# kelaendi/mused

Hardware: AMD Instinct MI355X
Metric: stream rows/sec, d=1024 l=128 window=10k synthetic (SWFD + kNN similarity + eigenstep + labels) (higher is better)
Workload: dtype f64; 1 GPU; synthetic d=1024 l=128 window=10000 k=50 (BASELINE config 2); stream=blob, W=10000, d=1024, l=128, k=50, modalities=1, swfd_levels=14, rccl_ranks=1, lanes_per_gpu=20, padded_window_slots=2

## Files before the change

mused_amd/csrc/swfd.hip:

```cpp
#include <vector>

#include "internal.h"

namespace mused {

struct Swfd {
  int N, d, ell, L, S, cap, n2, n4, n3;
  int lanes;
  double R;
  long i;
  int pend;
  long restart_mark;
  int skip_dead;
  bool twin;
  int sweeps;
  double* buf;
  double* queue;
  long long* qt;
  int* meta;
  int* rep;
  int* list;
  int* offs;
  int oround;
  int* kact;
  long long* ostat;
  long long* dropped;
  double* theta;
  double *T, *Wc;
  int gram_split;
  double* gpart;
  int* plan;
  int* keep_src;
  long long* now_dev;
  int* status;
  int* status_host;
  EigPlan* eig;
  double *stack, *Wq, *Bout, *sig_out, *qinfo;
  int* qsel;
  EigPlan* eigq;
  EigPlan* eigq3;
  int pre_chunk;
  double *pre_in, *pre_out, *pre_gram;
  EigPlan* eigp;
};

static inline int sk_index(const Swfd* h, int lane, int level, int kind) { return lane * 2 * h->L + kind * h->L + level; }

struct BitWord { unsigned long long w; };
template <typename T>
__device__ __forceinline__ double row_elem(const T* row, int c) { return (double)row[c]; }
template <>
__device__ __forceinline__ double row_elem<BitWord>(const BitWord* row, int c) {
  return (double)((row[c >> 6].w >> (c & 63)) & 1ull);
}

template <typename T>
__global__ void swfd_append_kernel(const T* __restrict__ X, long ldx, long lane_stride, int per_lane, int m, int d,
                                   int n2, int pend, const int* __restrict__ meta, double* __restrict__ buf) {
  const int r = blockIdx.x, s = blockIdx.y;
  X += (long)(s / per_lane) * lane_stride;
  const int row = meta[s * 4 + 0] + pend + r;
  if (row >= n2) return;
  double* dst = buf + ((long)s * n2 + row) * d;
  const T* src = X + (long)r * ldx;
  for (int c = threadIdx.x; c < d; c += blockDim.x) dst[c] = row_elem<T>(src, c);
}

__global__ void swfd_restart_kernel(double* __restrict__ buf, double* __restrict__ queue, long long* __restrict__ qt,
                                    int* __restrict__ meta, long long* __restrict__ dropped, int L, long buf_elems,
                                    long queue_elems, int cap) {
  const int lane = blockIdx.y / L, j = blockIdx.y - lane * L;
  const int sm = lane * 2 * L + j, sa = sm + L;
  const long gid = (long)blockIdx.x * blockDim.x + threadIdx.x;
  if (gid < buf_elems) {
    buf[sm * buf_elems + gid] = buf[sa * buf_elems + gid];
    buf[sa * buf_elems + gid] = 0.0;
  }
  if (gid < queue_elems) queue[sm * queue_elems + gid] = queue[sa * queue_elems + gid];
  if (gid < cap) qt[sm * cap + gid] = qt[sa * cap + gid];
  if (gid == 0) {
    for (int k = 0; k < 4; ++k) {
      meta[sm * 4 + k] = meta[sa * 4 + k];
      meta[sa * 4 + k] = 0;
    }
    dropped[sm] = dropped[sa];
    dropped[sa] = 0;
  }
}

__global__ void swfd_set_now_kernel(long long* now, long long v) { *now = v; }

constexpr int SWFD_OFFS_ROUND = 16;
__global__ __launch_bounds__(1024) void swfd_rep_kernel(const int* __restrict__ meta, int L, int nchains, int* __restrict__ rep,
                                                        int twin, const long long* __restrict__ dropped, long long epoch_start,
                                                        int skip_dead, long long* __restrict__ now_dev, long long now, int pend,
                                                        int ell, int n2, int* __restrict__ list, int* __restrict__ offs,
                                                        int* __restrict__ kact, long long* __restrict__ ostat, int oround) {
  extern __shared__ int s_key[];
  __shared__ int s_hist[17];
  const int t = threadIdx.x, S = nchains * L;
  if (t == 0) *now_dev = now;
  if (t < 17) s_hist[t] = 0;
  auto put = [&](int s, int r) {
    rep[s] = r;
    const int na = meta[s * 4 + 0] + pend;
    s_key[s] = (r == s) ? (na < n2 ? na : n2) : -1;
  };
  for (int c = t; c < nchains; c += 1024) {
    const int base = ((twin && (c & 1)) ? c - 1 : c) * L;
    if (twin && (c & 1)) {
      int r = base + L - 1;
      put(c * L + L - 1, r);
      for (int j = L - 2; j >= 0; --j) {
        if (meta[(base + j) * 4 + 3] != 0) r = base + j;
        put(c * L + j, r);
      }
      continue;
    }
    const bool dead_ok = skip_dead && !twin && (c & 1) == 0;
    int r = base + L - 1;
    put(r, r);
    for (int j = L - 2; j >= 0; --j) {
      if (meta[(base + j) * 4 + 3] != 0) r = base + j;
      put(base + j, (dead_ok && dropped[base + j] > epoch_start) ? -1 : r);
    }
  }
  __syncthreads();
  if (!list) return;
  for (int s = t; s < S; s += 1024) {
    const int key = s_key[s];
    if (key < 0) continue;
    int rank = 0;
    for (int j = 0; j < S; ++j) {
      const int kj = s_key[j];
      rank += (kj > key) || (kj == key && j < s);
    }
    list[1 + rank] = s;
    const int n = offs ? n2 - ((n2 - (key > ell ? key : ell)) & ~(oround - 1)) : n2;
    if (offs) offs[s] = n2 - n;
    if (kact) kact[s] = min(n2, (key + 15) & ~15);
    atomicAdd(&s_hist[16], 1);
    atomicAdd(&s_hist[(n - 1) >> 4 < 16 ? (n - 1) >> 4 : 15], 1);
  }
  __syncthreads();
  if (t == 0) list[0] = s_hist[16];
  if (t == 0) ostat[0] += 1;
  if (t == 1) ostat[1] += s_hist[16];
  if (t < 16) ostat[2 + t] += s_hist[t];
}

__global__ __launch_bounds__(1024) void swfd_decide_kernel(const double* __restrict__ evals,
                                                          const double* __restrict__ U, int ldu, int n2,
                                                          int ell, int cap,
                                                          int N, const long long* __restrict__ now_p,
                                                          const double* __restrict__ theta, int* __restrict__ meta,
                                                          long long* __restrict__ qt, long long* __restrict__ dropped,
                                                          int* __restrict__ plan, int* __restrict__ keep_src,
                                                          double* __restrict__ Wc, const int* __restrict__ rep) {
  __shared__ double lam[1024];
  __shared__ int order[1024];
  __shared__ double scale[512];
  const int s = blockIdx.x, t = threadIdx.x;
  const long long now = *now_p;
  const int sr = rep ? rep[s] : s;
  if (sr < 0) return;
  const double* ev = evals + (long)sr * ldu;
  const double* Us = U + (long)sr * ldu * ldu;
  if (t < n2) lam[t] = ev[t];
  __syncthreads();
  if (t < n2) {
    const double mine = lam[t];
    int rank = 0;
    for (int j = 0; j < n2; ++j) {
      const double o = lam[j];
      rank += (o > mine) || (o == mine && j < t);
    }
    order[rank] = t;
  }
  __syncthreads();
  __shared__ int s_part[16];
  __shared__ int s_wcnt[3][4];
  const int head0 = meta[s * 4 + 1], cnt0 = meta[s * 4 + 2];
  long long* q = qt + (long)s * cap;
  const int wv = t >> 6, ln = t & 63;
  int expired = 0;
  for (int k = t; k < cnt0; k += 1024) expired += (q[(head0 + k) % cap] + N <= now) ? 1 : 0;
#pragma unroll
  for (int o = 32; o > 0; o >>= 1) expired += __shfl_xor(expired, o);
  if (ln == 0) s_part[wv] = expired;
  __syncthreads();
  int nexp = 0;
#pragma unroll
  for (int ww = 0; ww < 16; ++ww) nexp += s_part[ww];
  const int head1 = (head0 + nexp) % cap, cnt1 = cnt0 - nexp;
  const double l0 = lam[order[0]];
  const double delta = lam[order[ell - 1]] > 0.0 ? lam[order[ell - 1]] : 0.0;
  const double tol = 1e-10 * (l0 > 0.0 ? l0 : 0.0);
  const double th = theta[s];
  int kind = 0, near = 0;
  double sc = 0.0;
  if (t < ell) {
    const double l = lam[order[t]];
    double s2 = l - delta;
    s2 = s2 > 0.0 ? s2 : 0.0;
    if (s2 > tol) {
      sc = sqrt(s2 / l) / l;
      kind = (s2 >= th) ? 2 : 1;
      near = (kind == 2 && s2 < 2.0 * th) ? 1 : 0;
    }
    scale[t] = sc;
  }
  const unsigned long long mk = __ballot(kind == 1), md = __ballot(kind == 2), mn = __ballot(near != 0);
  const unsigned long long below = (ln == 0) ? 0ull : (~0ull >> (64 - ln));
  if (ln == 0 && wv < 4) {
    s_wcnt[0][wv] = __popcll(mk);
    s_wcnt[1][wv] = __popcll(md);
    s_wcnt[2][wv] = __popcll(mn);
  }
  __syncthreads();
  int kpos = __popcll(mk & below), dpos = __popcll(md & below);
  int nk = 0, nd = 0, nnear = 0;
#pragma unroll
  for (int ww = 0; ww < 4; ++ww) {
    if (ww < wv) {
      kpos += s_wcnt[0][ww];
      dpos += s_wcnt[1][ww];
    }
    nk += s_wcnt[0][ww];
    nd += s_wcnt[1][ww];
    nnear += s_wcnt[2][ww];
  }
  const int nevict = (cnt1 + nd > cap) ? (cnt1 + nd - cap) : 0;
  if (t == 0) {
    long long drop = dropped[s];
    if (nevict > 0) {
      const long long ts = q[(head1 + nevict - 1) % cap];
      drop = ts > drop ? ts : drop;
    }
    dropped[s] = drop;
  }
  __syncthreads();
  if (t < ell) {
    int pos = 0;
    if (kind == 1) {
      pos = kpos;
      keep_src[s * ell + kpos] = t;
    } else if (kind == 2) {
      pos = (head1 + cnt1 + dpos) % cap;
      q[pos] = now;
    }
    plan[(s * ell + t) * 2 + 0] = kind;
    plan[(s * ell + t) * 2 + 1] = pos;
  }
  if (t == 0) {
    meta[s * 4 + 0] = nk;
    meta[s * 4 + 1] = (head1 + nevict) % cap;
    meta[s * 4 + 2] = cnt1 + nd - nevict;
    meta[s * 4 + 3] += nnear;
  }
  __syncthreads();
  if (sr != s) return;
  double* W = Wc + (long)s * ell * n2;
  for (int e = t; e < ell * n2; e += 1024) {
    const int i = e / n2, a = e - i * n2;
    const double sc = scale[i];
    W[e] = (sc != 0.0) ? sc * Us[(long)order[i] * ldu + a] : 0.0;
  }
}

__global__ void swfd_scatter_kernel(const double* __restrict__ T, const int* __restrict__ plan,
                                    const int* __restrict__ keep_src, const int* __restrict__ meta,
                                    double* __restrict__ buf, double* __restrict__ queue, int n2, int ell, int cap,
                                    int d, const int* __restrict__ rep) {
  const int rho = blockIdx.x, s = blockIdx.y;
  if (rep && rep[s] < 0) return;
  const double* Ts = T + (long)(rep ? rep[s] : s) * ell * d;
  if (rho < ell && plan[(s * ell + rho) * 2] == 2) {
    const int slot = plan[(s * ell + rho) * 2 + 1];
    double* dst = queue + ((long)s * cap + slot) * d;
    const double* src = Ts + (long)rho * d;
    for (int c = threadIdx.x; c < d; c += blockDim.x) dst[c] = src[c];
  }
  const int nk = meta[s * 4 + 0];
  double* dst = buf + ((long)s * n2 + rho) * d;
  if (rho < nk) {
    const double* src = Ts + (long)keep_src[s * ell + rho] * d;
    for (int c = threadIdx.x; c < d; c += blockDim.x) dst[c] = src[c];
  } else {
    for (int c = threadIdx.x; c < d; c += blockDim.x) dst[c] = 0.0;
  }
}

static int swfd_rotate_all(Swfd* h, hipStream_t st) {
  const int S = h->S, n2 = h->n2, d = h->d, ell = h->ell;
  int rc;
  if (h->rep)
    hipLaunchKernelGGL(swfd_rep_kernel, dim3(1), dim3(1024), sizeof(int) * (size_t)S, st, h->meta, h->L, 2 * h->lanes, h->rep,
                       h->twin ? 1 : 0, h->dropped, (long long)(((h->i - 1) / h->N) * h->N), h->skip_dead, h->now_dev,
                       (long long)h->i, h->pend, ell, n2, h->list, h->offs, h->kact, h->ostat, h->oround);
  else
    hipLaunchKernelGGL(swfd_set_now_kernel, dim3(1), dim3(1), 0, st, h->now_dev, (long long)h->i);
  if (h->gram_split > 1) {
    const int kchunk = ((d + h->gram_split - 1) / h->gram_split + 15) / 16 * 16;
    if ((rc = gemm_f64_batched_splitk(true, true, h->buf, d, (long)n2 * d, h->buf, d, (long)n2 * d, h->gpart, n2, n2, d, S, kchunk,
                                      h->gram_split, st, h->rep, h->list)))
      return rc;
    if ((rc = gemm_batched_splitk_reduce(h->gpart, h->gram_split, (long)n2 * n2, eig_plan_input(h->eig), S, h->rep, st, h->list)))
      return rc;
  } else if ((rc = gemm_f64(true, true, h->buf, d, (long)n2 * d, h->buf, d, (long)n2 * d, eig_plan_input(h->eig), n2,
                            (long)n2 * n2, n2, n2, d, S, 1.0, st, h->rep, h->list)))
    return rc;
  if ((rc = eig_plan_run_inplace(h->eig, nullptr, nullptr, st, true))) return rc;
  const EigColumns e = eig_plan_columns(h->eig);
  hipLaunchKernelGGL(swfd_decide_kernel, dim3(S), dim3(1024), 0, st, e.lam, e.cols, e.ld, n2, ell, h->cap, h->N, h->now_dev,
                     h->theta, h->meta, h->qt, h->dropped, h->plan, h->keep_src, h->Wc, h->rep);
  if ((rc = gemm_f64(true, false, h->Wc, n2, (long)ell * n2, h->buf, d, (long)n2 * d, h->T, d, (long)ell * d, ell, d,
                     n2, S, 1.0, st, h->rep, h->list, h->kact)))
    return rc;
  hipLaunchKernelGGL(swfd_scatter_kernel, dim3(n2, S), dim3(256), 0, st, h->T, h->plan, h->keep_src, h->meta, h->buf,
                     h->queue, n2, ell, h->cap, d, h->rep);
  MUSED_LAUNCH_CHECK();
  h->pend = 0;
  return MUSED_OK;
}

static int swfd_restart(Swfd* h, hipStream_t st) {
  const long be = (long)h->n2 * h->d, qe = (long)h->cap * h->d;
  const long m = be > qe ? be : qe;
  hipLaunchKernelGGL(swfd_restart_kernel, dim3(cdiv(m, 256), h->L * h->lanes), dim3(256), 0, st, h->buf, h->queue, h->qt,
                     h->meta, h->dropped, h->L, be, qe, h->cap);
  MUSED_LAUNCH_CHECK();
  return MUSED_OK;
}

constexpr int SWFD_PRE_MAX = 96;
struct PreBlocks {
  int row0[SWFD_PRE_MAX];
  int rows[SWFD_PRE_MAX];
};

template <typename T>
__global__ void swfd_pre_load_kernel(const T* __restrict__ X, long ldx, long lane_stride, int lanes, int ell, int d,
                                     PreBlocks pb, double* __restrict__ out) {
  const int row = blockIdx.x, z = blockIdx.y;
  const int blk = z / lanes, lane = z - blk * lanes;
  double* dst = out + ((long)z * ell + row) * d;
  if (row < pb.rows[blk]) {
    const T* src = X + (long)lane * lane_stride + (long)(pb.row0[blk] + row) * ldx;
    for (int c = threadIdx.x; c < d; c += blockDim.x) dst[c] = row_elem<T>(src, c);
  } else {
    for (int c = threadIdx.x; c < d; c += blockDim.x) dst[c] = 0.0;
  }
}

__global__ void swfd_pre_pack_kernel(const double* __restrict__ gram, int ell, double* __restrict__ Gc) {
  const int n2 = 2 * ell;
  const long z = blockIdx.y;
  const long e = (long)blockIdx.x * blockDim.x + threadIdx.x;
  if (e >= (long)n2 * n2) return;
  const int col = (int)(e / n2), row = (int)(e - (long)col * n2);
  double v = 0.0;
  if (col < ell) v = (row < ell) ? gram[z * ell * ell + (long)col * ell + row] : ((row - ell == col) ? 1.0 : 0.0);
  Gc[z * n2 * n2 + e] = v;
}

template <typename T>
static int swfd_prerotate(Swfd* h, const T* X, long ldx, long lane_stride, const PreBlocks& pb, int nblk, hipStream_t st) {
  const int ell = h->ell, d = h->d, B = h->lanes, n2 = h->n2;
  int rc;
  const int Z = nblk * B;
  hipLaunchKernelGGL(swfd_pre_load_kernel<T>, dim3(ell, Z), dim3(256), 0, st, X, ldx, lane_stride, B, ell, d, pb,
                     h->pre_in);
  if ((rc = gemm_f64(true, true, h->pre_in, d, (long)ell * d, h->pre_in, d, (long)ell * d, h->pre_gram, ell,
                     (long)ell * ell, ell, ell, d, Z, 1.0, st)))
    return rc;
  hipLaunchKernelGGL(swfd_pre_pack_kernel, dim3(cdiv((long)n2 * n2, 256), Z), dim3(256), 0, st, h->pre_gram, ell,
                     eig_plan_input(h->eigp));
  if ((rc = eig_plan_run_inplace(h->eigp, nullptr, nullptr, st, true))) return rc;
  const double* cols = eig_plan_columns(h->eigp).cols;
  const int ld = eig_plan_columns(h->eigp).ld;
  if ((rc = gemm_f64(true, false, cols + ell, ld, (long)ld * ld, h->pre_in, d, (long)ell * d, h->pre_out, d, (long)ell * d,
                     ell, d, ell, Z, 1.0, st)))
    return rc;
  MUSED_LAUNCH_CHECK();
  return MUSED_OK;
}

template <typename T>
static int swfd_append_t(Swfd* h, const T* X, long ldx, long lane_stride, long m, hipStream_t st) {
  long r = 0;
  int rc;
  PreBlocks pb;
  int pre_n = 0, pre_next = 0;
  while (r < m) {
    if (h->i > 0 && h->i % h->N == 0 && h->restart_mark != h->i) {
      if ((rc = swfd_restart(h, st))) return rc;
      h->restart_mark = h->i;
      h->twin = false;
    }
    const long in_epoch = h->i % h->N;
    long until = h->ell - (in_epoch % h->ell);
    if (h->N - in_epoch < until) until = h->N - in_epoch;
    const long take = (m - r) < until ? (m - r) : until;
    bool from_pre = false;
    if (h->pre_chunk > 0 && h->pend == 0 && take == until) {
      if (pre_next >= pre_n) {
        pre_n = pre_next = 0;
        long rr = r, ii = h->i;
        while (pre_n < h->pre_chunk && rr < m) {
          const long ie = ii % h->N;
          long u = h->ell - (ie % h->ell);
          if (h->N - ie < u) u = h->N - ie;
          if (m - rr < u) break;
          pb.row0[pre_n] = (int)rr;
          pb.rows[pre_n] = (int)u;
          ++pre_n;
          rr += u;
          ii += u;
        }
        if ((rc = swfd_prerotate<T>(h, X, ldx, lane_stride, pb, pre_n, st))) return rc;
      }
      from_pre = true;
    }
    if (from_pre) {
      const double* src = h->pre_out + (long)pre_next * h->lanes * h->ell * h->d;
      hipLaunchKernelGGL(swfd_append_kernel<double>, dim3((int)take, h->S), dim3(256), 0, st, src, (long)h->d,
                         (long)h->ell * h->d, 2 * h->L, (int)take, h->d, h->n2, h->pend, h->meta, h->buf);
      ++pre_next;
    } else {
      hipLaunchKernelGGL(swfd_append_kernel<T>, dim3((int)take, h->S), dim3(256), 0, st, X + r * ldx, ldx, lane_stride,
                         2 * h->L, (int)take, h->d, h->n2, h->pend, h->meta, h->buf);
    }
    MUSED_LAUNCH_CHECK();
    h->pend += (int)take;
    h->i += take;
    r += take;
    if (take == until) {
      if ((rc = swfd_rotate_all(h, st))) return rc;
    }
  }
  return MUSED_OK;
}

__global__ void swfd_select_kernel(const int* __restrict__ meta, const long long* __restrict__ qt,
                                   const long long* __restrict__ dropped, int L, int cap, int N, long long now,
                                   int* __restrict__ qsel_all) {
  if (threadIdx.x != 0) return;
  const int lane = blockIdx.x;
  const int base = lane * 2 * L;
  int* qsel = qsel_all + (long)lane * (4 + cap);
  int lvl = L - 1;
  for (int j = 0; j < L; ++j) {
    const long long dr = dropped[base + j];
    if (dr == 0 || dr + N <= now) { lvl = j; break; }
  }
  const int sk = base + lvl;
  const int head = meta[sk * 4 + 1], cnt = meta[sk * 4 + 2];
  int ns = 0;
  for (int q = 0; q < cnt; ++q) {
    const int slot = (head + q) % cap;
    if (qt[(long)sk * cap + slot] + N > now) qsel[4 + ns++] = slot;
  }
  qsel[0] = lvl;
  qsel[1] = ns;
  qsel[2] = meta[sk * 4 + 0];
  qsel[3] = sk;
}

__global__ void swfd_stack_kernel(const int* __restrict__ qsel_all, const double* __restrict__ buf,
                                  const double* __restrict__ queue, int n2, int n4, int cap, int d, int pend,
                                  double* __restrict__ stack) {
  const int rho = blockIdx.x, lane = blockIdx.y;
  const int* qsel = qsel_all + (long)lane * (4 + cap);
  const int ns = qsel[1], nk = qsel[2], sk = qsel[3];
  const double* src = nullptr;
  if (rho < ns) src = queue + ((long)sk * cap + qsel[4 + rho]) * d;
  else if (rho < ns + nk + pend) src = buf + ((long)sk * n2 + (rho - ns)) * d;
  double* dst = stack + ((long)lane * n4 + rho) * d;
  for (int c = threadIdx.x; c < d; c += blockDim.x) dst[c] = src ? src[c] : 0.0;
}

__global__ __launch_bounds__(1024) void swfd_decide_query_kernel(const double* __restrict__ evals_all,
                                                                const double* __restrict__ U_all, int ldu, int n4, int ell,
                                                                int cap, const int* __restrict__ qsel_all,
                                                                double* __restrict__ Wq_all,
                                                                double* __restrict__ qinfo_all) {
  __shared__ double lam[1024];
  __shared__ int order[1024];
  __shared__ double scale[512];
  const int t = threadIdx.x, lane = blockIdx.x;
  const double* evals = evals_all + (long)lane * ldu;
  const double* U = U_all + (long)lane * ldu * ldu;
  const int* qsel = qsel_all + (long)lane * (4 + cap);
  double* Wq = Wq_all + (long)lane * ell * n4;
  double* qinfo = qinfo_all + (long)lane * 2;
  if (t < n4) lam[t] = evals[t];
  __syncthreads();
  if (t < n4) {
    const double mine = lam[t];
    int rank = 0;
    for (int j = 0; j < n4; ++j) {
      const double o = lam[j];
      rank += (o > mine) || (o == mine && j < t);
    }
    order[rank] = t;
  }
  __syncthreads();
  const double l0 = lam[order[0]];
  const double delta = lam[order[ell - 1]] > 0.0 ? lam[order[ell - 1]] : 0.0;
  const double tol = 1e-10 * (l0 > 0.0 ? l0 : 0.0);
  if (t < ell) {
    const double l = lam[order[t]];
    double s2 = l - delta;
    s2 = s2 > 0.0 ? s2 : 0.0;
    scale[t] = (s2 > tol) ? sqrt(s2 / l) / l : 0.0;
  }
  if (t == 0) {
    qinfo[0] = (double)qsel[0];
    qinfo[1] = delta;
  }
  __syncthreads();
  for (int e = t; e < ell * n4; e += 1024) {
    const int i = e / n4, a = e - i * n4;
    const double sc = scale[i];
    Wq[e] = (sc != 0.0) ? sc * U[(long)order[i] * ldu + a] : 0.0;
  }
}

__global__ __launch_bounds__(256) void swfd_finish_rows_kernel(double* __restrict__ B, int d, double* __restrict__ sig) {
  __shared__ double sv[4];
  __shared__ int si[4];
  __shared__ double ss[4];
  __shared__ double s_sign;
  const long rowid = (long)blockIdx.y * gridDim.x + blockIdx.x;
  double* row = B + rowid * d;
  double best = -1.0, sq = 0.0;
  int bi = 0x7fffffff;
  for (int c = threadIdx.x; c < d; c += 256) {
    const double v = row[c];
    const double a = fabs(v);
    sq += v * v;
    if (a > best || (a == best && c < bi)) { best = a; bi = c; }
  }
#pragma unroll
  for (int o = 32; o > 0; o >>= 1) {
    const double ob = __shfl_xor(best, o);
    const int oi = __shfl_xor(bi, o);
    sq += __shfl_xor(sq, o);
    if (ob > best || (ob == best && oi < bi)) { best = ob; bi = oi; }
  }
  if ((threadIdx.x & 63) == 0) { sv[threadIdx.x >> 6] = best; si[threadIdx.x >> 6] = bi; ss[threadIdx.x >> 6] = sq; }
  __syncthreads();
  if (threadIdx.x == 0) {
    for (int w = 1; w < 4; ++w)
      if (sv[w] > best || (sv[w] == best && si[w] < bi)) { best = sv[w]; bi = si[w]; }
    s_sign = (row[bi] < 0.0) ? -1.0 : 1.0;
    sig[rowid] = sqrt(ss[0] + ss[1] + ss[2] + ss[3]);
  }
  __syncthreads();
  if (s_sign < 0.0)
    for (int c = threadIdx.x; c < d; c += 256) row[c] = -row[c];
}

static int swfd_query(Swfd* h, double* outB, double* outSigma, double* outInfo, hipStream_t st) {
  const bool small = (h->pend == 0) && h->eigq3;
  EigPlan* const eq = small ? h->eigq3 : h->eigq;
  const int n4 = small ? h->n3 : h->n4, d = h->d, ell = h->ell, B = h->lanes;
  int rc;
  hipLaunchKernelGGL(swfd_select_kernel, dim3(B), dim3(64), 0, st, h->meta, h->qt, h->dropped, h->L, h->cap, h->N,
                     (long long)h->i, h->qsel);
  hipLaunchKernelGGL(swfd_stack_kernel, dim3(n4, B), dim3(256), 0, st, h->qsel, h->buf, h->queue, h->n2, n4, h->cap, d,
                     h->pend, h->stack);
  if ((rc = gemm_f64(true, true, h->stack, d, (long)n4 * d, h->stack, d, (long)n4 * d, eig_plan_input(eq), n4,
                     (long)n4 * n4, n4, n4, d, B, 1.0, st)))
    return rc;
  if ((rc = eig_plan_run_inplace(eq, nullptr, nullptr, st, true))) return rc;
  const EigColumns e = eig_plan_columns(eq);
  hipLaunchKernelGGL(swfd_decide_query_kernel, dim3(B), dim3(1024), 0, st, e.lam, e.cols, e.ld, n4, ell, h->cap, h->qsel, h->Wq,
                     h->qinfo);
  if ((rc = gemm_f64(true, false, h->Wq, n4, (long)ell * n4, h->stack, d, (long)n4 * d, h->Bout, d, (long)ell * d, ell,
                     d, n4, B, 1.0, st)))
    return rc;
  hipLaunchKernelGGL(swfd_finish_rows_kernel, dim3(ell, B), dim3(256), 0, st, h->Bout, d, h->sig_out);
  MUSED_LAUNCH_CHECK();
  MUSED_CHECK_HIP(hipMemcpyAsync(outB, h->Bout, sizeof(double) * (size_t)B * ell * d, hipMemcpyDeviceToDevice, st));
  if (outSigma)
    MUSED_CHECK_HIP(hipMemcpyAsync(outSigma, h->sig_out, sizeof(double) * (size_t)B * ell, hipMemcpyDeviceToDevice, st));
  if (outInfo) MUSED_CHECK_HIP(hipMemcpyAsync(outInfo, h->qinfo, sizeof(double) * 2 * B, hipMemcpyDeviceToDevice, st));
  return MUSED_OK;
}

static size_t swfd_half_bytes(const Swfd* h) {
  const size_t L = h->L;
  return L * ((size_t)h->n2 * h->d * 8 + (size_t)h->cap * h->d * 8 + (size_t)h->cap * 8 + 4 * 4 + 8);
}

}

using namespace mused;

extern "C" {

int mused_swfd_create_lanes(long N, double R, int d, int ell, int sweeps, int lanes, void** out);
int mused_swfd_destroy(void* handle);

int mused_swfd_create(long N, double R, int d, int ell, int sweeps, void** out) {
  return mused_swfd_create_lanes(N, R, d, ell, sweeps, 1, out);
}

static int swfd_create_impl(Swfd* h, long N, double R, int d, int ell, int sweeps, int lanes);

int mused_swfd_create_lanes(long N, double R, int d, int ell, int sweeps, int lanes, void** out) {
  MUSED_REQUIRE(out && N >= 1 && d >= 1 && ell >= 1 && ell <= 256, "mused_swfd_create: need N, d >= 1 and 1 <= sketch_dim <= 256");
  MUSED_REQUIRE(lanes >= 1 && lanes <= 64, "mused_swfd_create_lanes: 1 <= lanes <= 64");
  MUSED_REQUIRE(N < (1l << 31), "mused_swfd_create: N too large");
  CaptureLock resource_guard(capture_mutex());
  Swfd* h = new Swfd();
  memset(h, 0, sizeof(*h));
  const int rc = swfd_create_impl(h, N, R, d, ell, sweeps, lanes);
  if (rc) {
    (void)mused_swfd_destroy(h);
    return rc;
  }
  *out = h;
  return MUSED_OK;
}

static int swfd_create_impl(Swfd* h, long N, double R, int d, int ell, int sweeps, int lanes) {
  h->N = (int)N; h->R = R; h->d = d; h->ell = ell;
  double r1 = R > 1.0 ? R : 1.0;
  int lg = 0;
  while ((double)(1ull << lg) < r1 && lg < 62) ++lg;
  h->L = lg + 1;
  h->lanes = lanes;
  h->S = 2 * h->L * lanes;
  MUSED_REQUIRE(h->S <= 8192, "mused_swfd_create: %d sketches (lanes x 2 levels), at most 8192", h->S);
  h->cap = 2 * ell;
  h->n2 = 2 * ell;
  h->n4 = 4 * ell;
  h->n3 = (3 * ell + 1) & ~1;
  h->sweeps = sweeps > 0 ? sweeps : 24;
  h->restart_mark = -1;
  h->twin = true;
  const size_t S = h->S, n2 = h->n2, n4 = h->n4, cap = h->cap, dd = d, l = ell;
#define ALLOC(p, bytes) MUSED_CHECK_HIP(hipMalloc((void**)&(p), (bytes)))
#define ZALLOC(p, bytes) do { ALLOC(p, bytes); MUSED_CHECK_HIP(hipMemset((p), 0, (bytes))); } while (0)
  ZALLOC(h->buf, 8 * S * n2 * dd);
  ZALLOC(h->queue, 8 * S * cap * dd);
  ZALLOC(h->qt, 8 * S * cap);
  ZALLOC(h->meta, 4 * S * 4);
  {
    const char* dd = getenv("MUSED_SWFD_DEDUPE");
    if (!(dd && dd[0] == '0')) ALLOC(h->rep, 4 * S);
    auto off = [](const char* name) { const char* v = getenv(name); return v && v[0] == '0'; };
    if (h->rep && !off("MUSED_SWFD_LIST")) {
      ZALLOC(h->list, 4 * (S + 1));
      ZALLOC(h->ostat, 8 * 18);
      if (!off("MUSED_SWFD_ORDERS")) ZALLOC(h->offs, 4 * S);
      const char* orr = getenv("MUSED_SWFD_ORDERS");
      const int rv = orr ? atoi(orr) : 0;
      h->oround = (rv == 1 || rv == 16 || rv == 32) ? rv : SWFD_OFFS_ROUND;
      if (!off("MUSED_SWFD_KACT")) ZALLOC(h->kact, 4 * S);
    }
    const char* sd = getenv("MUSED_SWFD_SKIP_DEAD");
    h->skip_dead = (sd && sd[0] == '0') ? 0 : 1;
  }
  ZALLOC(h->dropped, 8 * S);
  ZALLOC(h->status, 4);
  MUSED_CHECK_HIP(hipHostMalloc((void**)&h->status_host, sizeof(int), hipHostMallocDefault));
  ALLOC(h->theta, 8 * S);
  ALLOC(h->T, 8 * S * l * dd); ALLOC(h->Wc, 8 * S * l * n2);
  ALLOC(h->plan, 4 * S * l * 2); ALLOC(h->keep_src, 4 * S * l); ALLOC(h->now_dev, 8);
  {
    const char* gs = getenv("MUSED_SWFD_GRAM_SPLIT");
    h->gram_split = gs ? atoi(gs) : (d >= 8192 ? 8 : 1);
    if (h->gram_split < 1 || h->gram_split > 16) h->gram_split = 1;
    if (h->gram_split > 1) ALLOC(h->gpart, 8 * S * (size_t)h->gram_split * n2 * n2);
  }
  const size_t Bn = lanes;
  ALLOC(h->stack, 8 * Bn * n4 * dd);
  ALLOC(h->Wq, 8 * Bn * l * n4); ALLOC(h->Bout, 8 * Bn * l * dd); ALLOC(h->sig_out, 8 * Bn * l);
  ALLOC(h->qinfo, 8 * 2 * Bn); ALLOC(h->qsel, 4 * Bn * (4 + cap));
#undef ZALLOC
#undef ALLOC
  std::vector<double> th(S);
  for (int lane = 0; lane < lanes; ++lane)
    for (int kind = 0; kind < 2; ++kind)
      for (int j = 0; j < h->L; ++j) th[sk_index(h, lane, j, kind)] = ldexp((double)h->N / ell, j);
  MUSED_CHECK_HIP(hipMemcpy(h->theta, th.data(), 8 * S, hipMemcpyHostToDevice));
  int rc;
  if ((rc = gemm_f64_prepare_all())) return rc;
  if ((rc = eig_plan_create(h->n2, h->S, h->sweeps, true, &h->eig, h->rep, EIG_PLAN_TOP_HALF, h->status, 0, h->list, h->offs)))
    return rc;
  if ((rc = eig_plan_create(h->n4, lanes, h->sweeps + 2, true, &h->eigq, nullptr, EIG_PLAN_TOP_FD, h->status, ell))) return rc;
  if (h->n3 < h->n4 &&
      (rc = eig_plan_create(h->n3, lanes, h->sweeps + 2, true, &h->eigq3, nullptr, EIG_PLAN_TOP_FD, h->status, ell)))
    return rc;
  {
    const char* pr = getenv("MUSED_SWFD_PREROT");
    const bool want_pre = pr ? (pr[0] != '0') : !eig_plan_direct_solver(h->eig);
    if (want_pre) {
      const size_t per_block = (size_t)lanes * ell * dd * 8;
      size_t c = ((size_t)256 << 20) / per_block;
      c = c < 1 ? 1 : (c > (size_t)SWFD_PRE_MAX ? (size_t)SWFD_PRE_MAX : c);
      h->pre_chunk = (int)c;
      MUSED_CHECK_HIP(hipMalloc((void**)&h->pre_in, c * per_block));
      MUSED_CHECK_HIP(hipMalloc((void**)&h->pre_out, c * per_block));
      MUSED_CHECK_HIP(hipMalloc((void**)&h->pre_gram, 8 * c * lanes * l * l));
      const char* ps = getenv("MUSED_SWFD_PREROT_SWEEPS");
      const int psw = ps ? atoi(ps) : 5;
      if ((rc = eig_plan_create(h->n2, (int)c * lanes, psw > 0 ? psw : 5, true, &h->eigp, nullptr,
                                EIG_PLAN_FIXED_SWEEPS | EIG_PLAN_NO_SORT, h->status)))
        return rc;
    }
  }
  return MUSED_OK;
}

int mused_swfd_destroy(void* handle) {
  Swfd* h = (Swfd*)handle;
  if (!h) return MUSED_OK;
  CaptureLock resource_guard(capture_mutex());
  eig_plan_destroy(h->eig);
  eig_plan_destroy(h->eigq);
  if (h->eigq3) eig_plan_destroy(h->eigq3);
  if (h->eigp) eig_plan_destroy(h->eigp);
  void* bufs[] = {h->buf, h->queue, h->qt, h->meta, h->dropped, h->theta, h->T, h->Wc, h->plan,
                  h->keep_src, h->now_dev, h->stack, h->Wq, h->Bout, h->sig_out, h->qinfo, h->qsel,
                  h->rep, h->pre_in, h->pre_out, h->pre_gram, h->status, h->gpart, h->list, h->offs, h->kact, h->ostat};
  for (void* b : bufs) (void)hipFree(b);
  if (h->status_host) (void)hipHostFree(h->status_host);
  delete h;
  return MUSED_OK;
}

int mused_swfd_levels(void* handle) { return handle ? ((Swfd*)handle)->L : -1; }

int mused_swfd_profile(void* handle, int on) {
  Swfd* h = (Swfd*)handle;
  MUSED_REQUIRE(h, "mused_swfd_profile: null handle");
  return eig_plan_profile(h->eig, on != 0);
}

int mused_swfd_profile_read(void* handle, double* total_ms, long* launches, double* bytes_per_launch) {
  Swfd* h = (Swfd*)handle;
  MUSED_REQUIRE(h && total_ms && launches && bytes_per_launch, "mused_swfd_profile_read: null pointer");
  return eig_plan_profile_read(h->eig, total_ms, launches, bytes_per_launch);
}

extern "C" int mused_swfd_profile_read_direct(void* handle, double* total_ms, long* launches, double* matrices_solved,
                                              int* direct, double* tridiag_ms) {
  Swfd* h = (Swfd*)handle;
  MUSED_REQUIRE(h && total_ms && launches && matrices_solved && direct, "mused_swfd_profile_read_direct: null pointer");
  *direct = eig_plan_direct_solver(h->eig) ? 1 : 0;
  return eig_plan_profile_read_direct(h->eig, total_ms, launches, matrices_solved, tridiag_ms);
}

int mused_swfd_append_lanes(void* handle, const void* rows, int dtype, long n_rows, long ld, long lane_stride,
                            void* stream);

int mused_swfd_append(void* handle, const void* rows, int dtype, long n_rows, long ld, void* stream) {
  Swfd* h = (Swfd*)handle;
  MUSED_REQUIRE(h && h->lanes == 1, "mused_swfd_append: this handle has %d lanes, use mused_swfd_append_lanes", h ? h->lanes : 0);
  return mused_swfd_append_lanes(handle, rows, dtype, n_rows, ld, 0, stream);
}

int mused_swfd_append_lanes(void* handle, const void* rows, int dtype, long n_rows, long ld, long lane_stride,
                            void* stream) {
  Swfd* h = (Swfd*)handle;
  MUSED_REQUIRE(h && (rows || n_rows == 0) && n_rows >= 0, "mused_swfd_append: bad arguments");
  hipStream_t st = (hipStream_t)stream;
  if (dtype == MUSED_BITS) {
    MUSED_REQUIRE(ld >= (h->d + 63) / 64, "mused_swfd_append: bit rows need a pitch of at least ceil(d / 64) words");
    return swfd_append_t<BitWord>(h, (const BitWord*)rows, ld, lane_stride, n_rows, st);
  }
  MUSED_REQUIRE(ld >= h->d, "mused_swfd_append: row pitch smaller than d");
  if (dtype == MUSED_F32) return swfd_append_t<float>(h, (const float*)rows, ld, lane_stride, n_rows, st);
  if (dtype == MUSED_F64) return swfd_append_t<double>(h, (const double*)rows, ld, lane_stride, n_rows, st);
  if (dtype == MUSED_I64) return swfd_append_t<long long>(h, (const long long*)rows, ld, lane_stride, n_rows, st);
  set_error("mused_swfd_append: unsupported dtype %d", dtype);
  return MUSED_ERR_UNSUPPORTED;
}

int mused_swfd_lanes(void* handle) { return handle ? ((Swfd*)handle)->lanes : -1; }

int mused_swfd_debug_state(void* handle, int* rep_out, int* meta_out) {
  Swfd* h = (Swfd*)handle;
  if (!h) return MUSED_ERR_ARG;
  MUSED_CHECK_HIP(hipDeviceSynchronize());
  if (h->rep && rep_out) MUSED_CHECK_HIP(hipMemcpy(rep_out, h->rep, 4 * (size_t)h->S, hipMemcpyDeviceToHost));
  if (meta_out) MUSED_CHECK_HIP(hipMemcpy(meta_out, h->meta, 16 * (size_t)h->S, hipMemcpyDeviceToHost));
  return h->rep ? 1 : 0;
}

int mused_swfd_debug_orders(void* handle, long long* out) {
  Swfd* h = (Swfd*)handle;
  if (!h || !out) return MUSED_ERR_ARG;
  if (!h->ostat) return 0;
  MUSED_CHECK_HIP(hipDeviceSynchronize());
  MUSED_CHECK_HIP(hipMemcpy(out, h->ostat, 8 * 18, hipMemcpyDeviceToHost));
  return 1;
}

int mused_swfd_query(void* handle, double* out_sketch, double* out_sigma, double* out_info, void* stream) {
  Swfd* h = (Swfd*)handle;
  MUSED_REQUIRE(h && out_sketch, "mused_swfd_query: null pointer");
  return swfd_query(h, out_sketch, out_sigma, out_info, (hipStream_t)stream);
}

int mused_swfd_status(void* handle, int* status_out, void* stream) {
  Swfd* h = (Swfd*)handle;
  MUSED_REQUIRE(h && status_out, "mused_swfd_status: null pointer");
  MUSED_CHECK_HIP(hipMemcpyAsync(h->status_host, h->status, sizeof(int), hipMemcpyDeviceToHost, (hipStream_t)stream));
  MUSED_CHECK_HIP(hipStreamSynchronize((hipStream_t)stream));
  *status_out = *h->status_host;
  return MUSED_OK;
}

int mused_swfd_counters(void* handle, long* rows_seen, int* pending) {
  Swfd* h = (Swfd*)handle;
  MUSED_REQUIRE(h && rows_seen && pending, "mused_swfd_counters: null pointer");
  *rows_seen = h->i;
  *pending = h->pend;
  return MUSED_OK;
}

long mused_swfd_half_bytes(void* handle) { return handle ? (long)swfd_half_bytes((Swfd*)handle) : -1; }

static int half_copy(Swfd* h, int kind, char* blob, bool to_blob, hipStream_t st) {
  const size_t L = h->L;
  const size_t o = (size_t)kind * L;
  struct Part { char* dev; size_t bytes; };
  Part parts[5] = {
      {(char*)(h->buf + o * h->n2 * h->d), L * h->n2 * h->d * 8},
      {(char*)(h->queue + o * h->cap * h->d), L * (size_t)h->cap * h->d * 8},
      {(char*)(h->qt + o * h->cap), L * (size_t)h->cap * 8},
      {(char*)(h->meta + o * 4), L * 16},
      {(char*)(h->dropped + o), L * 8},
  };
  size_t off = 0;
  for (const Part& p : parts) {
    if (to_blob) MUSED_CHECK_HIP(hipMemcpyAsync(blob + off, p.dev, p.bytes, hipMemcpyDeviceToDevice, st));
    else MUSED_CHECK_HIP(hipMemcpyAsync(p.dev, blob + off, p.bytes, hipMemcpyDeviceToDevice, st));
    off += p.bytes;
  }
  return MUSED_OK;
}

int mused_swfd_export_half(void* handle, int kind, void* dst, void* stream) {
  Swfd* h = (Swfd*)handle;
  MUSED_REQUIRE(h && dst && (kind == 0 || kind == 1), "mused_swfd_export_half: bad arguments");
  MUSED_REQUIRE(h->lanes == 1, "mused_swfd_export_half: single-lane handles only");
  return half_copy(h, kind, (char*)dst, true, (hipStream_t)stream);
}

int mused_swfd_import_half(void* handle, int kind, const void* src, void* stream) {
  Swfd* h = (Swfd*)handle;
  MUSED_REQUIRE(h && src && (kind == 0 || kind == 1), "mused_swfd_import_half: bad arguments");
  MUSED_REQUIRE(h->lanes == 1, "mused_swfd_import_half: single-lane handles only");
  h->twin = false;
  return half_copy(h, kind, (char*)src, false, (hipStream_t)stream);
}

int mused_swfd_begin_epoch(void* handle, long rows_seen, const void* main_half, void* stream) {
  Swfd* h = (Swfd*)handle;
  MUSED_REQUIRE(h && rows_seen >= 0 && rows_seen % h->N == 0, "mused_swfd_begin_epoch: rows_seen must be a multiple of N");
  MUSED_REQUIRE(!main_half || h->lanes == 1, "mused_swfd_begin_epoch: a state blob can only be imported into a single-lane handle");
  hipStream_t st = (hipStream_t)stream;
  const size_t S = h->S, L = h->L;
  MUSED_CHECK_HIP(hipMemsetAsync(h->buf, 0, 8 * S * (size_t)h->n2 * h->d, st));
  MUSED_CHECK_HIP(hipMemsetAsync(h->meta, 0, 4 * S * 4, st));
  MUSED_CHECK_HIP(hipMemsetAsync(h->dropped, 0, 8 * S, st));
  MUSED_CHECK_HIP(hipMemsetAsync(h->qt, 0, 8 * S * h->cap, st));
  (void)L;
  if (main_half) {
    int rc = half_copy(h, 0, (char*)main_half, false, st);
    if (rc) return rc;
  }
  h->i = rows_seen;
  h->pend = 0;
  h->restart_mark = rows_seen;
  h->twin = (main_half == nullptr);
  return MUSED_OK;
}

}

extern "C" int mused_fd_rotate(double* buf, int ell, int d, double* sigma_out, int sweeps, void* stream) {
  MUSED_REQUIRE(buf && sigma_out && ell >= 1 && d >= 1, "mused_fd_rotate: bad arguments");
  void* hv = nullptr;
  int rc = mused_swfd_create(1l << 30, 1.0, d, ell, sweeps, &hv);
  if (rc) return rc;
  mused::Swfd* h = (mused::Swfd*)hv;
  hipStream_t st = (hipStream_t)stream;
  const size_t bytes = sizeof(double) * (size_t)2 * ell * d;
  hipError_t e = hipMemcpyAsync(h->buf, buf, bytes, hipMemcpyDeviceToDevice, st);
  h->i = 2 * ell;
  h->pend = 2 * ell;
  if (e == hipSuccess) rc = mused::swfd_rotate_all(h, st);
  if (e == hipSuccess && !rc) e = hipMemcpyAsync(buf, h->buf, bytes, hipMemcpyDeviceToDevice, st);
  if (e == hipSuccess && !rc) {
    hipLaunchKernelGGL(mused::swfd_finish_rows_kernel, dim3(ell), dim3(256), 0, st, buf, d, sigma_out);
    e = hipStreamSynchronize(st);
  }
  mused_swfd_destroy(hv);
  if (rc) return rc;
  MUSED_CHECK_HIP(e);
  return MUSED_OK;
}
```

Baseline: 613,000 rows/s.

## Fuse next-block append into SWFD scatter and zero only previously used rows

Adds a settle kernel that replaces the post-rotation scatter. It writes kept sketch rows, then directly copies the next block of incoming rows into the buffer, which removes the separate append launch for that block. It zeroes only up to the previously used row count instead of the whole tail, and row copies are vectorised with double2 loads and stores. Dead replicas still get their incoming rows placed. This adds bookkeeping (used counts, tail_dirty flags, a placed-rows check) and a risk of stale rows if the dirty tracking is wrong.

```diff
diff --git a/mused_amd/csrc/swfd.hip b/mused_amd/csrc/swfd.hip
--- a/mused_amd/csrc/swfd.hip
+++ b/mused_amd/csrc/swfd.hip
@@ -15,6 +15,9 @@
   bool twin;
   int sweeps;
   double* buf;
+  bool tail_dirty;
+  bool settle;
+  int* used;
   double* queue;
   long long* qt;
   int* meta;
@@ -55,15 +58,57 @@
 }
 
 template <typename T>
+__device__ __forceinline__ double2 row_pair(const T* row, int c);
+template <>
+__device__ __forceinline__ double2 row_pair<double>(const double* row, int c) { return *(const double2*)(row + c); }
+template <>
+__device__ __forceinline__ double2 row_pair<long long>(const long long* row, int c) {
+  const longlong2 v = *(const longlong2*)(row + c);
+  return make_double2((double)v.x, (double)v.y);
+}
+template <>
+__device__ __forceinline__ double2 row_pair<float>(const float* row, int c) {
+  const float2 v = *(const float2*)(row + c);
+  return make_double2((double)v.x, (double)v.y);
+}
+template <>
+__device__ __forceinline__ double2 row_pair<BitWord>(const BitWord* row, int c) {
+  const unsigned long long w = row[c >> 6].w >> (c & 63);
+  return make_double2((double)(w & 1ull), (double)((w >> 1) & 1ull));
+}
+template <typename T> struct RowPairAlign { static constexpr unsigned long long mask = 15; };
+template <> struct RowPairAlign<float> { static constexpr unsigned long long mask = 7; };
+template <> struct RowPairAlign<BitWord> { static constexpr unsigned long long mask = 7; };
+
+template <typename T>
+__device__ __forceinline__ void row_copy(double* __restrict__ dst, const T* __restrict__ src, int d) {
+  const bool wide = (d & 1) == 0 && ((unsigned long long)dst & 15ull) == 0 &&
+                    ((unsigned long long)src & RowPairAlign<T>::mask) == 0;
+  if (wide) {
+    double2* dst2 = (double2*)dst;
+    for (int c = threadIdx.x; c < (d >> 1); c += blockDim.x) dst2[c] = row_pair<T>(src, 2 * c);
+  } else {
+    for (int c = threadIdx.x; c < d; c += blockDim.x) dst[c] = row_elem<T>(src, c);
+  }
+}
+
+__device__ __forceinline__ void row_zero(double* __restrict__ dst, int d) {
+  if ((d & 1) == 0 && ((unsigned long long)dst & 15ull) == 0) {
+    double2* dst2 = (double2*)dst;
+    for (int c = threadIdx.x; c < (d >> 1); c += blockDim.x) dst2[c] = make_double2(0.0, 0.0);
+  } else {
+    for (int c = threadIdx.x; c < d; c += blockDim.x) dst[c] = 0.0;
+  }
+}
+
+template <typename T>
 __global__ void swfd_append_kernel(const T* __restrict__ X, long ldx, long lane_stride, int per_lane, int m, int d,
                                    int n2, int pend, const int* __restrict__ meta, double* __restrict__ buf) {
   const int r = blockIdx.x, s = blockIdx.y;
   X += (long)(s / per_lane) * lane_stride;
   const int row = meta[s * 4 + 0] + pend + r;
   if (row >= n2) return;
-  double* dst = buf + ((long)s * n2 + row) * d;
-  const T* src = X + (long)r * ldx;
-  for (int c = threadIdx.x; c < d; c += blockDim.x) dst[c] = row_elem<T>(src, c);
+  row_copy<T>(buf + ((long)s * n2 + row) * d, X + (long)r * ldx, d);
 }
 
 __global__ void swfd_restart_kernel(double* __restrict__ buf, double* __restrict__ queue, long long* __restrict__ qt,
@@ -156,7 +201,8 @@
                                                           const double* __restrict__ theta, int* __restrict__ meta,
                                                           long long* __restrict__ qt, long long* __restrict__ dropped,
                                                           int* __restrict__ plan, int* __restrict__ keep_src,
-                                                          double* __restrict__ Wc, const int* __restrict__ rep) {
+                                                          double* __restrict__ Wc, const int* __restrict__ rep,
+                                                          int* __restrict__ used, int pend) {
   __shared__ double lam[1024];
   __shared__ int order[1024];
   __shared__ double scale[512];
@@ -253,6 +299,7 @@
     plan[(s * ell + t) * 2 + 1] = pos;
   }
   if (t == 0) {
+    if (used) used[s] = min(n2, meta[s * 4 + 0] + pend);
     meta[s * 4 + 0] = nk;
     meta[s * 4 + 1] = (head1 + nevict) % cap;
     meta[s * 4 + 2] = cnt1 + nd - nevict;
@@ -291,7 +338,37 @@
   }
 }
 
-static int swfd_rotate_all(Swfd* h, hipStream_t st) {
+template <typename Src>
+__global__ void swfd_settle_kernel(const double* __restrict__ T, const int* __restrict__ plan,
+                                   const int* __restrict__ keep_src, const int* __restrict__ meta,
+                                   const int* __restrict__ used, int fill_all, double* __restrict__ buf,
+                                   double* __restrict__ queue, int n2, int ell, int cap, int d, const int* __restrict__ rep,
+                                   const Src* __restrict__ X, long ldx, long lane_stride, int per_lane, int nxt) {
+  const int rho = blockIdx.x, s = blockIdx.y;
+  const int sr = rep ? rep[s] : s;
+  const int nk = meta[s * 4 + 0];
+  if (sr < 0) {
+    if (rho < nxt && nk + rho < n2)
+      row_copy<Src>(buf + ((long)s * n2 + nk + rho) * d, X + (long)(s / per_lane) * lane_stride + (long)rho * ldx, d);
+    return;
+  }
+  const double* Ts = T + (long)sr * ell * d;
+  if (rho < ell && plan[(s * ell + rho) * 2] == 2) {
+    const int slot = plan[(s * ell + rho) * 2 + 1];
+    row_copy<double>(queue + ((long)s * cap + slot) * d, Ts + (long)rho * d, d);
+  }
+  double* dst = buf + ((long)s * n2 + rho) * d;
+  if (rho < nk) {
+    row_copy<double>(dst, Ts + (long)keep_src[s * ell + rho] * d, d);
+  } else if (rho < nk + nxt) {
+    row_copy<Src>(dst, X + (long)(s / per_lane) * lane_stride + (long)(rho - nk) * ldx, d);
+  } else if (rho < (fill_all ? n2 : used[s])) {
+    row_zero(dst, d);
+  }
+}
+
+template <typename Src>
+static int swfd_rotate_all(Swfd* h, hipStream_t st, const Src* next, long ldx, long lane_stride, int nxt) {
   const int S = h->S, n2 = h->n2, d = h->d, ell = h->ell;
   int rc;
   if (h->rep)
@@ -313,12 +390,20 @@
   if ((rc = eig_plan_run_inplace(h->eig, nullptr, nullptr, st, true))) return rc;
   const EigColumns e = eig_plan_columns(h->eig);
   hipLaunchKernelGGL(swfd_decide_kernel, dim3(S), dim3(1024), 0, st, e.lam, e.cols, e.ld, n2, ell, h->cap, h->N, h->now_dev,
-                     h->theta, h->meta, h->qt, h->dropped, h->plan, h->keep_src, h->Wc, h->rep);
+                     h->theta, h->meta, h->qt, h->dropped, h->plan, h->keep_src, h->Wc, h->rep, h->settle ? h->used : nullptr,
+                     h->pend);
   if ((rc = gemm_f64(true, false, h->Wc, n2, (long)ell * n2, h->buf, d, (long)n2 * d, h->T, d, (long)ell * d, ell, d,
                      n2, S, 1.0, st, h->rep, h->list, h->kact)))
     return rc;
-  hipLaunchKernelGGL(swfd_scatter_kernel, dim3(n2, S), dim3(256), 0, st, h->T, h->plan, h->keep_src, h->meta, h->buf,
-                     h->queue, n2, ell, h->cap, d, h->rep);
+  if (h->settle) {
+    hipLaunchKernelGGL(swfd_settle_kernel<Src>, dim3(n2, S), dim3(256), 0, st, h->T, h->plan, h->keep_src, h->meta, h->used,
+                       h->tail_dirty ? 1 : 0, h->buf, h->queue, n2, ell, h->cap, d, h->rep, next, ldx, lane_stride, 2 * h->L,
+                       nxt);
+    h->tail_dirty = false;
+  } else {
+    hipLaunchKernelGGL(swfd_scatter_kernel, dim3(n2, S), dim3(256), 0, st, h->T, h->plan, h->keep_src, h->meta, h->buf,
+                       h->queue, n2, ell, h->cap, d, h->rep);
+  }
   MUSED_LAUNCH_CHECK();
   h->pend = 0;
   return MUSED_OK;
@@ -392,6 +477,7 @@
   int rc;
   PreBlocks pb;
   int pre_n = 0, pre_next = 0;
+  int placed = 0;
   while (r < m) {
     if (h->i > 0 && h->i % h->N == 0 && h->restart_mark != h->i) {
       if ((rc = swfd_restart(h, st))) return rc;
@@ -422,7 +508,13 @@
       }
       from_pre = true;
     }
-    if (from_pre) {
+    if (placed > 0) {
+      if (placed != take) {
+        set_error("mused_swfd_append: internal: %d rows placed ahead, the block takes %ld", placed, take);
+        return MUSED_ERR_STATE;
+      }
+      placed = 0;
+    } else if (from_pre) {
       const double* src = h->pre_out + (long)pre_next * h->lanes * h->ell * h->d;
       hipLaunchKernelGGL(swfd_append_kernel<double>, dim3((int)take, h->S), dim3(256), 0, st, src, (long)h->d,
                          (long)h->ell * h->d, 2 * h->L, (int)take, h->d, h->n2, h->pend, h->meta, h->buf);
@@ -436,7 +528,15 @@
     h->i += take;
     r += take;
     if (take == until) {
-      if ((rc = swfd_rotate_all(h, st))) return rc;
+      long nxt = 0;
+      if (h->settle && h->pre_chunk == 0 && r < m && h->i % h->N != 0) {
+        const long ie = h->i % h->N;
+        long u = h->ell - (ie % h->ell);
+        if (h->N - ie < u) u = h->N - ie;
+        nxt = (m - r) < u ? (m - r) : u;
+      }
+      if ((rc = swfd_rotate_all<T>(h, st, nxt ? X + r * ldx : nullptr, ldx, lane_stride, (int)nxt))) return rc;
+      placed = (int)nxt;
     }
   }
   return MUSED_OK;
@@ -664,6 +764,8 @@
     }
     const char* sd = getenv("MUSED_SWFD_SKIP_DEAD");
     h->skip_dead = (sd && sd[0] == '0') ? 0 : 1;
+    h->settle = !off("MUSED_SWFD_SETTLE");
+    if (h->settle) ZALLOC(h->used, 4 * S);
   }
   ZALLOC(h->dropped, 8 * S);
   ZALLOC(h->status, 4);
@@ -727,7 +829,7 @@
   if (h->eigp) eig_plan_destroy(h->eigp);
   void* bufs[] = {h->buf, h->queue, h->qt, h->meta, h->dropped, h->theta, h->T, h->Wc, h->plan,
                   h->keep_src, h->now_dev, h->stack, h->Wq, h->Bout, h->sig_out, h->qinfo, h->qsel,
-                  h->rep, h->pre_in, h->pre_out, h->pre_gram, h->status, h->gpart, h->list, h->offs, h->kact, h->ostat};
+                  h->rep, h->pre_in, h->pre_out, h->pre_gram, h->status, h->gpart, h->list, h->offs, h->kact, h->ostat, h->used};
   for (void* b : bufs) (void)hipFree(b);
   if (h->status_host) (void)hipHostFree(h->status_host);
   delete h;
@@ -791,6 +893,15 @@
   if (h->rep && rep_out) MUSED_CHECK_HIP(hipMemcpy(rep_out, h->rep, 4 * (size_t)h->S, hipMemcpyDeviceToHost));
   if (meta_out) MUSED_CHECK_HIP(hipMemcpy(meta_out, h->meta, 16 * (size_t)h->S, hipMemcpyDeviceToHost));
   return h->rep ? 1 : 0;
+}
+
+int mused_swfd_debug_used(void* handle, int* used_out) {
+  Swfd* h = (Swfd*)handle;
+  if (!h || !used_out) return MUSED_ERR_ARG;
+  if (!h->used) return 0;
+  MUSED_CHECK_HIP(hipDeviceSynchronize());
+  MUSED_CHECK_HIP(hipMemcpy(used_out, h->used, 4 * (size_t)h->S, hipMemcpyDeviceToHost));
+  return 1;
 }
 
 int mused_swfd_debug_orders(void* handle, long long* out) {
@@ -859,6 +970,7 @@
   MUSED_REQUIRE(h && src && (kind == 0 || kind == 1), "mused_swfd_import_half: bad arguments");
   MUSED_REQUIRE(h->lanes == 1, "mused_swfd_import_half: single-lane handles only");
   h->twin = false;
+  h->tail_dirty = true;
   return half_copy(h, kind, (char*)src, false, (hipStream_t)stream);
 }
 
@@ -881,6 +993,7 @@
   h->pend = 0;
   h->restart_mark = rows_seen;
   h->twin = (main_half == nullptr);
+  h->tail_dirty = (main_half != nullptr);
   return MUSED_OK;
 }
 
@@ -897,7 +1010,7 @@
   hipError_t e = hipMemcpyAsync(h->buf, buf, bytes, hipMemcpyDeviceToDevice, st);
   h->i = 2 * ell;
   h->pend = 2 * ell;
-  if (e == hipSuccess) rc = mused::swfd_rotate_all(h, st);
+  if (e == hipSuccess) rc = mused::swfd_rotate_all<double>(h, st, nullptr, 0, 0, 0);
   if (e == hipSuccess && !rc) e = hipMemcpyAsync(buf, h->buf, bytes, hipMemcpyDeviceToDevice, st);
   if (e == hipSuccess && !rc) {
     hipLaunchKernelGGL(mused::swfd_finish_rows_kernel, dim3(ell), dim3(256), 0, st, buf, d, sigma_out);
```

Measured after the change: 625,500 rows/s, median of 6. +2.0%, better.
